# AnjieCheng/SpatialRGPT

Measured on AMD Instinct MI355X. Metric: region-grounded output tokens/sec @ VILA1.5-8B, 8 regions, greedy, higher is better.
Workload: dtype bf16; 1 GPU; BASELINE configs[1]: SpatialRGPT-VILA1.5-8B geometry (Llama-3-8B 32L/4096/GQA-8 + SigLIP-so400m 384px x2 passes + regiongpt extractor + mlp_downsample), 8 region masks, bs=1 per GPU, prompt 64 ids -> T=259, greedy 128 new tokens; parallelism=dp1, decode=hipGraph, llm_weights=bf16

## Files before the change

### include/srgpt.h

```cpp
#ifndef SRGPT_H_
#define SRGPT_H_

#include <stddef.h>
#include <stdint.h>

#ifdef __cplusplus
extern "C" {
#endif

typedef void* srgpt_stream_t;

enum { SRGPT_F32 = 0, SRGPT_BF16 = 1 };
enum { SRGPT_ACT_NONE = 0, SRGPT_ACT_GELU_ERF = 1, SRGPT_ACT_GELU_TANH = 2, SRGPT_ACT_SILU = 3, SRGPT_ACT_QUICK_GELU = 4 };
enum {
  SRGPT_OK = 0,
  SRGPT_ERR_ARG = -1,
  SRGPT_ERR_UNSUPPORTED = -2,
  SRGPT_ERR_LAUNCH = -3,
  SRGPT_ERR_STATE = -4
};
enum {
  SRGPT_OUT_PLAIN = 0,
  SRGPT_OUT_DECONV2X = 1
};
// ... 13 lines not shown
                    int64_t ws_bytes, int norm_kind, const void* norm_w, const void* norm_b, void* Y, float norm_eps, int dtype,
                    srgpt_stream_t stream);

int srgpt_gemm_swiglu(const void* A, const void* Wgu, void* out, int M, int I, int K, void* gu_scratch, void* ws,
                      int64_t ws_bytes, int dtype, srgpt_stream_t stream);

int srgpt_gemm_rope_kv_append(const void* A, const void* W, void* qkv, int K, void* ws, int64_t ws_bytes, void* kcache,
                              void* vcache, const int* pos0, const void* cos_tab, const void* sin_tab, int B, int T, int Hq,
                              int Hkv, int D, int max_pos, int dtype, srgpt_stream_t stream);

int srgpt_gemm_w8(const void* A, const void* W8, const float* wscale, const void* bias, const void* residual, void* C,
                  int M, int N, int K, int lda, int ldc, int act, int out_f32, void* ws, int64_t ws_bytes,
                  srgpt_stream_t stream);

int srgpt_quant_rows_e4m3(const void* x, void* q, float* scale, int M, int K, int ldx, srgpt_stream_t stream);
int srgpt_quant_rows_e4m3_rmsnorm(const void* x, const void* norm_w, float eps, void* q, float* scale, int M, int K, int ldx,
                                  srgpt_stream_t stream);
int srgpt_quant_rows_e4m3_swiglu(const void* gate_up, void* q, float* scale, int M, int inter, srgpt_stream_t stream);
int srgpt_gemm_w8a8(const void* A8, const float* ascale, const void* W8, const float* wscale, const void* bias,
                    const void* residual, void* C, int M, int N, int K, int lda, int ldc, int out_f32, void* ws,
                    int64_t ws_bytes, srgpt_stream_t stream);

int srgpt_gemv(const void* x, const void* W, const void* norm_w, float norm_eps, const void* residual,
               void* out, int batch, int N, int K, int swiglu, int out_f32, int dtype, srgpt_stream_t stream);
int srgpt_gemv_w8(const void* x, const void* W8, const float* wscale, const void* norm_w, float norm_eps,
                  const void* residual, void* out, int batch, int N, int K, int swiglu, int out_f32,
                  srgpt_stream_t stream);
#define SRGPT_ROWSS_STRIDE 512
int srgpt_gemv_rowss_supported(int batch, int dtype, int fp8);
int srgpt_gemv_rowss(const void* x, const void* W, const void* W8, const float* wscale, const void* norm_w, float norm_eps,
                     const void* residual, void* out, int batch, int N, int K, int swiglu, int out_f32, const float* rowss_in,
                     float* rowss_out, int packed_rows, srgpt_stream_t stream);
size_t srgpt_packed_bytes(int N, int K, int elem_bytes, int rows);
int srgpt_pack_decode_weights(const void* W, void* out, int N, int K, int elem_bytes, int rows, srgpt_stream_t stream);

int srgpt_layernorm(const void* x, const void* w, const void* b, void* y, int rows, int cols, float eps,
                    int act, int dtype, srgpt_stream_t stream);
int srgpt_rmsnorm(const void* x, const void* w, void* y, int rows, int cols, float eps, int dtype,
                  srgpt_stream_t stream);

int srgpt_attention(const void* q, const void* k, const void* v, void* o, int B, int Tq, int Tk, int Hq,
                    int Hkv, int D, int64_t q_bs, int64_t q_ts, int64_t q_hs, int64_t k_bs, int64_t k_ts,
                    int64_t k_hs, int64_t v_bs, int64_t v_ts, int64_t v_hs, float scale, int causal,
                    const int* kv_len, int dtype, srgpt_stream_t stream);

int srgpt_rope_kv_append(void* qkv, void* kcache, void* vcache, const int* pos0, const void* cos_tab,
                         const void* sin_tab, int B, int T, int Hq, int Hkv, int D, int max_pos, int dtype,
                         srgpt_stream_t stream);

int64_t srgpt_decode_attn_ws_floats(int B, int Hq, int D);
int srgpt_decode_attention(const void* qkv, void* kcache, void* vcache, const int* pos, const void* cos_tab,
                           const void* sin_tab, void* out, float* ws, int B, int Hq, int Hkv, int D,
                           int max_pos, int dtype, srgpt_stream_t stream);

int64_t srgpt_region_pool_ws_floats(int M, int fw, int C);
int srgpt_region_pool(const void* feat, const void* masks, void* out, float* ws, int M, int mh, int mw,
                      int fw, int C, float rscale_h, float rscale_w, int mask_dtype, int dtype,
                      srgpt_stream_t stream);
int srgpt_region_pool_u8(const void* feat, const void* masks_u8, const int* ys, const int* xs, void* out, float* ws, int M,
                         int rh, int rw, int mh, int mw, int fw, int C, float rscale_h, float rscale_w, int dtype,
                         srgpt_stream_t stream);
int srgpt_avgpool(const void* x, void* y, int n_img, int in_w, int out_w, int C, int dtype,
                  srgpt_stream_t stream);
int srgpt_s2d(const void* x, void* y, int n_img, int g, int C, int dtype, srgpt_stream_t stream);
int srgpt_im2col(const void* images, void* out, int n_img, int S, int patch, int kp, int dtype,
                 srgpt_stream_t stream);

int srgpt_embed_rows(const void* table, const int64_t* ids, void* out, int n, int cols, int dtype,
                     srgpt_stream_t stream);
#define SRGPT_SPLICE_STATS 8
int64_t srgpt_splice_scratch_ints(int B, int n_images_total);
int srgpt_splice_plan(const int64_t* ids, const unsigned char* attn_mask, int B, int P, int nimg_feat, int n_images_total,
                      const int* img_info, int use_masks, int use_depths, int64_t mask_id, int64_t depth_id, int max_len, int Tcap,
                      int* desc, int* stats, int* scratch, srgpt_stream_t stream);
int srgpt_splice_gather(const int* desc, const int* stats, int B, int Tcap, int T, int left_pad, int cols, int dtype,
                        const void* embed, const void* image_features, const void* mask_embeds, const void* depth_embeds,
                        const int64_t* labels, int P, int64_t ignore_index, void* out, int64_t* labels_out,
                        unsigned char* attn_mask_out, srgpt_stream_t stream);
int srgpt_kv_beam_reorder(void* kcache, void* vcache, const int64_t* beam_idx, int layers, int batch, int num_beams, int kv_heads,
                          int max_pos, int head_dim, int live, int dtype, srgpt_stream_t stream);
int srgpt_scatter_rows(const void* src, const int* src_idx, const int* idx, void* dst, int n, int cols,
                       int dtype, srgpt_stream_t stream);
int srgpt_silu_mul(const void* gu, void* out, int rows, int inter, int dtype, srgpt_stream_t stream);
int srgpt_argmax(const float* logits, int64_t* ids_out, int B, int V, srgpt_stream_t stream);
int srgpt_cross_entropy(const float* logits, const int64_t* labels, float* row_loss, float* out, int rows, int V,
                        int64_t ignore_index, srgpt_stream_t stream);


typedef struct {
  float temperature;
  int top_k;
  float top_p;
  float top_p_rm;
  uint64_t seed;
  uint64_t counter;
  int* kept_out;
} srgpt_sampling;

int64_t srgpt_sample_ws_bytes(int B);
int srgpt_sample(const float* logits, srgpt_sampling* sp, int64_t* tok_out, void* ws, int B, int V, srgpt_stream_t stream);
int srgpt_sample_status(const void* ws, int B, srgpt_stream_t stream);
int64_t srgpt_sample_full_ws_bytes(int B, int V);
int srgpt_sample_full(const float* logits, srgpt_sampling* sp, int64_t* tok_out, uint32_t* kept_mask, void* ws, int B, int V,
                      srgpt_stream_t stream);

typedef struct {
// ... 122 lines not shown
```

### spatialrgpt_amd/_lib.py

```python
from __future__ import annotations

import ctypes as C
import os
from typing import Optional

_HERE = os.path.dirname(os.path.abspath(__file__))
LIB_PATH = os.path.join(_HERE, "libsrgpt_hip.so")

F32, BF16 = 0, 1
ACT_NONE, ACT_GELU_ERF, ACT_GELU_TANH, ACT_SILU, ACT_QUICK_GELU = 0, 1, 2, 3, 4
OUT_PLAIN, OUT_DECONV2X = 0, 1
ERR_ARG, ERR_UNSUPPORTED, ERR_LAUNCH, ERR_STATE = -1, -2, -3, -4

vp, i32, i64, f32 = C.c_void_p, C.c_int, C.c_int64, C.c_float


class VitWeights(C.Structure):
    _fields_ = [
        ("dtype", i32), ("hidden", i32), ("inter", i32), ("heads", i32), ("n_layers_run", i32),
        ("image_size", i32), ("patch", i32), ("kp", i32), ("inter_pad", i32), ("act", i32), ("eps", f32),
        ("patch_w", vp), ("patch_b", vp), ("pos_emb", vp), ("cls_emb", vp), ("pre_ln_w", vp), ("pre_ln_b", vp),
        ("ln1_w", C.POINTER(vp)), ("ln1_b", C.POINTER(vp)),
        ("wqkv", C.POINTER(vp)), ("bqkv", C.POINTER(vp)),
        ("wo", C.POINTER(vp)), ("bo", C.POINTER(vp)),
# ... 28 lines not shown


class Sampling(C.Structure):
    _fields_ = [("temperature", f32), ("top_k", i32), ("top_p", f32), ("top_p_rm", f32), ("seed", C.c_uint64),
                ("counter", C.c_uint64), ("kept_out", vp)]


class LogitsProc(C.Structure):
    _fields_ = [("repetition_penalty", f32), ("no_repeat_ngram", i32), ("min_new_tokens", i32), ("n_eos", i32), ("eos", i64 * 8)]


LOGITS_PROC_EOS_MAX = 8
LOGITS_PROC_HISTORY_MAX = 12288
SAMPLING_TOP_K_MAX = 64
SAMPLING_KEPT_MAX = 256
SAMPLING_VOCAB_MAX = 128 * 2048
SAMPLER_TOPK64, SAMPLER_FULL = 0, 1

NORM_RMS, NORM_LAYER = 1, 2
SPLICE_STATS = 8
ROWSS_STRIDE = 512
ABI_VERSION = 9

_SIGNATURES = {
    "srgpt_last_error": (C.c_char_p, []),
    "srgpt_abi_version": (i32, []),
    "srgpt_device_cus": (i32, []),
    "srgpt_gemm_ws_bytes": (i64, [i32, i32]),
    "srgpt_gemm": (i32, [vp, vp, vp, vp, vp, i32, i32, i32, i32, i32, i32, i32, i32, i32, i32, i32, vp, i64, i32, vp]),
    "srgpt_gemm_norm": (i32, [vp, vp, vp, vp, vp, i32, i32, i32, vp, i64, i32, vp, vp, vp, f32, i32, vp]),
    "srgpt_gemm_rope_kv_append": (i32, [vp, vp, vp, i32, vp, i64, vp, vp, vp, vp, vp, i32, i32, i32, i32, i32, i32, i32, vp]),
    "srgpt_gemm_swiglu": (i32, [vp, vp, vp, i32, i32, i32, vp, vp, i64, i32, vp]),
    "srgpt_gemm_w8": (i32, [vp, vp, vp, vp, vp, vp, i32, i32, i32, i32, i32, i32, i32, vp, i64, vp]),
    "srgpt_quant_rows_e4m3": (i32, [vp, vp, vp, i32, i32, i32, vp]),
    "srgpt_quant_rows_e4m3_rmsnorm": (i32, [vp, vp, f32, vp, vp, i32, i32, i32, vp]),
    "srgpt_quant_rows_e4m3_swiglu": (i32, [vp, vp, vp, i32, i32, vp]),
    "srgpt_gemm_w8a8": (i32, [vp, vp, vp, vp, vp, vp, vp, i32, i32, i32, i32, i32, i32, vp, i64, vp]),
    "srgpt_gemv": (i32, [vp, vp, vp, f32, vp, vp, i32, i32, i32, i32, i32, i32, vp]),
    "srgpt_gemv_w8": (i32, [vp, vp, vp, vp, f32, vp, vp, i32, i32, i32, i32, i32, vp]),
    "srgpt_splice_scratch_ints": (i64, [i32, i32]),
    "srgpt_splice_plan": (i32, [vp, vp, i32, i32, i32, i32, vp, i32, i32, i64, i64, i32, i32, vp, vp, vp, vp]),
    "srgpt_splice_gather": (i32, [vp, vp, i32, i32, i32, i32, i32, i32, vp, vp, vp, vp, vp, i32, i64, vp, vp, vp, vp]),
    "srgpt_gemv_rowss_supported": (i32, [i32, i32, i32]),
    "srgpt_gemv_rowss": (i32, [vp, vp, vp, vp, vp, f32, vp, vp, i32, i32, i32, i32, i32, vp, vp, i32, vp]),
    "srgpt_packed_bytes": (C.c_size_t, [i32, i32, i32, i32]),
    "srgpt_pack_decode_weights": (i32, [vp, vp, i32, i32, i32, i32, vp]),
    "srgpt_layernorm": (i32, [vp, vp, vp, vp, i32, i32, f32, i32, i32, vp]),
    "srgpt_rmsnorm": (i32, [vp, vp, vp, i32, i32, f32, i32, vp]),
    "srgpt_attention": (i32, [vp, vp, vp, vp, i32, i32, i32, i32, i32, i32, i64, i64, i64, i64, i64, i64, i64, i64,
                              i64, f32, i32, vp, i32, vp]),
    "srgpt_rope_kv_append": (i32, [vp, vp, vp, vp, vp, vp, i32, i32, i32, i32, i32, i32, i32, vp]),
    "srgpt_decode_attn_ws_floats": (i64, [i32, i32, i32]),
    "srgpt_decode_attention": (i32, [vp, vp, vp, vp, vp, vp, vp, vp, i32, i32, i32, i32, i32, i32, vp]),
    "srgpt_region_pool_ws_floats": (i64, [i32, i32, i32]),
    "srgpt_region_pool": (i32, [vp, vp, vp, vp, i32, i32, i32, i32, i32, f32, f32, i32, i32, vp]),
    "srgpt_region_pool_u8": (i32, [vp, vp, vp, vp, vp, vp, i32, i32, i32, i32, i32, i32, i32, f32, f32, i32, vp]),
    "srgpt_avgpool": (i32, [vp, vp, i32, i32, i32, i32, i32, vp]),
    "srgpt_s2d": (i32, [vp, vp, i32, i32, i32, i32, vp]),
    "srgpt_im2col": (i32, [vp, vp, i32, i32, i32, i32, i32, vp]),
    "srgpt_embed_rows": (i32, [vp, vp, vp, i32, i32, i32, vp]),
    "srgpt_kv_beam_reorder": (i32, [vp, vp, vp, i32, i32, i32, i32, i32, i32, i32, i32, vp]),
    "srgpt_scatter_rows": (i32, [vp, vp, vp, vp, i32, i32, i32, vp]),
    "srgpt_silu_mul": (i32, [vp, vp, i32, i32, i32, vp]),
    "srgpt_argmax": (i32, [vp, vp, i32, i32, vp]),
    "srgpt_cross_entropy": (i32, [vp, vp, vp, vp, i32, i32, i64, vp]),
    "srgpt_sample_ws_bytes": (i64, [i32]),
    "srgpt_sample": (i32, [vp, vp, vp, vp, i32, i32, vp]),
    "srgpt_sample_status": (i32, [vp, i32, vp]),
    "srgpt_sample_full_ws_bytes": (i64, [i32, i32]),
    "srgpt_sample_full": (i32, [vp, vp, vp, vp, vp, i32, i32, vp]),
    "srgpt_logits_process": (i32, [vp, vp, vp, i32, i32, vp, i32, i32, vp]),
    "srgpt_image_resize_normalize": (i32, [vp, i32, i32, i32, vp, vp, i32, vp, vp, i32, i32, i32, vp, vp, vp, vp, f32, i32, i32, vp]),
    "srgpt_mask_resize_nearest": (i32, [vp, i32, i32, i32, vp, vp, i32, i32, vp, i32, vp]),
    "srgpt_mask_pad_resize": (i32, [vp, i32, i32, i32, vp, vp, i32, vp, vp, i32, i32, i32, vp, vp, i32, vp]),
    "srgpt_vit_assemble_cls": (i32, [vp, vp, vp, vp, i32, i32, i32, i32, vp]),
    "srgpt_vit_ws_bytes": (i64, [C.POINTER(VitWeights), i32]),
    "srgpt_vit_forward": (i32, [C.POINTER(VitWeights), vp, vp, vp, i32, vp]),
    "srgpt_llm_ws_bytes": (i64, [C.POINTER(LlmWeights), i32, i32]),
    "srgpt_llm_prefill": (i32, [C.POINTER(LlmWeights), C.POINTER(LlmState), vp, i32, vp, vp, vp]),
    "srgpt_llm_prefill_ragged": (i32, [C.POINTER(LlmWeights), C.POINTER(LlmState), vp, i32, vp, vp, vp, vp]),
    "srgpt_llm_decode_step": (i32, [C.POINTER(LlmWeights), C.POINTER(LlmState), vp]),
    "srgpt_llm_sample_first": (i32, [C.POINTER(LlmWeights), C.POINTER(LlmState), vp]),
    "srgpt_llm_decode_sync_state": (i32, [C.POINTER(LlmWeights), C.POINTER(LlmState), vp]),
    "srgpt_llm_decode_graph_create": (i32, [C.POINTER(LlmWeights), C.POINTER(LlmState), vp, C.POINTER(vp)]),
    "srgpt_llm_sample_first_ex": (i32, [C.POINTER(LlmWeights), C.POINTER(LlmState), i32, vp]),
    "srgpt_llm_decode_step_ex": (i32, [C.POINTER(LlmWeights), C.POINTER(LlmState), i32, vp]),
    "srgpt_llm_decode_graph_create_ex": (i32, [C.POINTER(LlmWeights), C.POINTER(LlmState), i32, vp, C.POINTER(vp)]),
    "srgpt_llm_sample_first_proc": (i32, [C.POINTER(LlmWeights), C.POINTER(LlmState), i32, vp, vp]),
    "srgpt_llm_decode_step_proc": (i32, [C.POINTER(LlmWeights), C.POINTER(LlmState), i32, vp, vp]),
    "srgpt_llm_decode_graph_create_proc": (i32, [C.POINTER(LlmWeights), C.POINTER(LlmState), i32, vp, vp, C.POINTER(vp)]),
    "srgpt_graph_launch": (i32, [vp, i32, vp]),
    "srgpt_graph_destroy": (i32, [vp]),
}

EXPORTED_SYMBOLS = tuple(_SIGNATURES)

_lib: Optional[C.CDLL] = None


class SrgptNativeError(RuntimeError):
    pass


def load() -> C.CDLL:
    global _lib
    if _lib is not None:
# ... 37 lines not shown
```

### spatialrgpt_amd/csrc/attn.hip

```cpp
#include <stdlib.h>

#include <type_traits>

#include "attn_route.h"
#include "common.h"
#include "internal.h"

namespace {

template <typename T>
__global__ __launch_bounds__(64) void simple_attn_kernel(const T* __restrict__ q, const T* __restrict__ k,
                                                         const T* __restrict__ v, T* __restrict__ o, int Tq, int Tk,
                                                         int Hq, int Hkv, int D, int64_t q_bs, int64_t q_ts,
                                                         int64_t q_hs, int64_t k_bs, int64_t k_ts, int64_t k_hs,
                                                         int64_t v_bs, int64_t v_ts, int64_t v_hs, float scale,
                                                         int causal, const int* __restrict__ kv_len) {
  __shared__ float qs[256];
  const int t = blockIdx.x, h = blockIdx.y, b = blockIdx.z, lane = threadIdx.x;
  const int hk = h / (Hq / Hkv);
  const int klen = kv_len ? min(kv_len[b], Tk) : Tk;
  const T* qp = q + b * q_bs + (int64_t)t * q_ts + h * q_hs;
  for (int d = lane; d < D; d += 64) qs[d] = to_f(qp[d]);
  __syncthreads();
  const T* kb = k + b * k_bs + hk * k_hs;
// ... 473 lines not shown
    if (lq < G && g4 == 0) wm[wave][lq] = alpha;
    asm volatile("s_waitcnt lgkmcnt(0)" ::: "memory");
    __builtin_amdgcn_wave_barrier();
#pragma unroll
    for (int h = 0; h < G; ++h) {
      const float a_h = wm[wave][h];
      acc[h][0] *= a_h;
      acc[h][1] *= a_h;
    }
#pragma unroll
    for (int i = 0; i < 16; ++i) {
      const int key = kb + i;
      unsigned int vv = vreg[i];
      if (key == P) vv = vnw;
      if (key >= kend) vv = 0u;
      const float v0 = bf16lo(vv), v1 = bf16hi(vv);
#pragma unroll
      for (int h = 0; h < G; ++h) {
        const float ph = pw[wave][i][h];
        acc[h][0] = fmaf(ph, v0, acc[h][0]);
        acc[h][1] = fmaf(ph, v1, acc[h][1]);
      }
    }
    asm volatile("s_waitcnt lgkmcnt(0)" ::: "memory");
    __builtin_amdgcn_wave_barrier();
    if (kb + 64 < kend) fetch(kb + 64);
  }
  if (lq < G && g4 == 0) {
    wm[wave][lq] = m_run;
    wl[wave][lq] = l_run;
  }
#pragma unroll
  for (int h = 0; h < G; ++h) *reinterpret_cast<f32x2*>(&accs[wave][h][2 * lane]) = f32x2{acc[h][0], acc[h][1]};
  __syncthreads();
  float* wbase = ws + attn_ws_group(b, hk, Hkv, G, D);
  const PublishPartial publish;
  for (int w = tid; w < G * (D / 2); w += 256) {
    const int gq = w / (D / 2), d = 2 * (w - gq * (D / 2));
    const float M = fmaxf(fmaxf(wm[0][gq], wm[1][gq]), fmaxf(wm[2][gq], wm[3][gq]));
    float n0 = 0.f, n1 = 0.f, L = 0.f;
#pragma unroll
    for (int wv = 0; wv < 4; ++wv) {
      const float e = (wm[wv][gq] > -INFINITY) ? __expf(wm[wv][gq] - M) : 0.f;
      n0 = fmaf(e, accs[wv][gq][d], n0);
      n1 = fmaf(e, accs[wv][gq][d + 1], n1);
      L = fmaf(e, wl[wv][gq], L);
    }
    float* wp = wbase + attn_ws_row(gq, split, D);
    publish(wp + d, n0, n1);
    if (d == 0) publish(wp + D, M, L);
  }
  decode_ticket_merge<T, D, G, 64>(wbase, attn_ws_ticket(tickets, b, hk, Hkv), nlive, out + ((size_t)b * Hq + (size_t)hk * G) * D,
                                   &sc[0][0], stat_m, stat_l, tid, lane, wave);
}

template <typename T>
int launch_decode(const void* qkv, void* kc, void* vc, const int* pos, const void* ct, const void* st, void* out,
                  float* ws, int B, int Hq, int Hkv, int D, int max_pos, const DecodePrefetch& pf, hipStream_t s) {
  const AttnDecodeRoute r = attn_decode_route(std::is_same<T, bf16_t>::value, B, Hq, Hkv, D, max_pos, srgpt_device_cus());
  SRGPT_CHECK(r.status != ATTN_MAX_POS_TOO_LONG, SRGPT_ERR_UNSUPPORTED, "srgpt_decode_attention: max_pos %d exceeds %d cached positions",
              max_pos, ATTN_DEC_SPLIT_MAX * ATTN_DEC_CHUNK_MAX);
  SRGPT_CHECK(r.status != ATTN_BAD_HEAD_DIM, SRGPT_ERR_UNSUPPORTED, "srgpt_decode_attention: head_dim %d not supported (16,32,64,128)", D);
  SRGPT_CHECK(r.status != ATTN_BAD_GROUP, SRGPT_ERR_UNSUPPORTED, "srgpt_decode_attention: heads/kv_heads = %d not supported (1,2,4,8)",
              r.G);
  const float scale = 1.0f / sqrtf((float)D);
  int* tickets = reinterpret_cast<int*>(ws + attn_ws_partial_floats(B, Hq, D));
  const dim3 grid(r.n_attn + (pf.base ? pf.nblocks : 0)), block(256);
  int rc = SRGPT_OK;
  if constexpr (std::is_same<T, bf16_t>::value) {
    if (r.family == ATTN_DECODE_MFMA)
      rc = srgpt_switch<1, 2, 4, 8>(r.G, "heads/kv_heads", [&](auto g_c) {
        hipLaunchKernelGGL((decode_mfma_kernel<decltype(g_c)::value>), grid, block, 0, s, (const T*)qkv, (T*)kc, (T*)vc, pos,
                           (const T*)ct, (const T*)st, ws, tickets, (T*)out, Hq, Hkv, max_pos, r.nsplit, r.kpb, scale, r.n_attn, pf);
        return (int)SRGPT_OK;
      });
  }
  if (r.family == ATTN_DECODE_VALU)
    rc = srgpt_switch<16, 32, 64, 128>(D, "head_dim", [&](auto d_c) {
      return srgpt_switch<1, 2, 4, 8>(r.G, "heads/kv_heads", [&](auto g_c) {
        hipLaunchKernelGGL((decode_split_kernel<T, decltype(d_c)::value, decltype(g_c)::value>), grid, block, 0, s, (const T*)qkv,
                           (T*)kc, (T*)vc, pos, (const T*)ct, (const T*)st, ws, tickets, (T*)out, Hq, Hkv, max_pos, r.nsplit, scale,
                           r.n_attn, pf);
        return (int)SRGPT_OK;
      });
    });
  SRGPT_TRY(rc);
  SRGPT_LAUNCH_CHECK();
  return SRGPT_OK;
}

}

extern "C" int64_t srgpt_decode_attn_ws_floats(int B, int Hq, int D) {
  return (int64_t)attn_ws_floats(B, Hq, D);
}

int srgpt_decode_attention_pf(const void* qkv, void* kcache, void* vcache, const int* pos, const void* cos_tab,
                              const void* sin_tab, void* out, float* ws, int B, int Hq, int Hkv, int D, int max_pos, int dtype,
                              const void* next_w, int next_n, int next_k, int next_fp8, srgpt_stream_t stream) {
  SRGPT_CHECK(qkv && kcache && vcache && pos && cos_tab && sin_tab && out && ws, SRGPT_ERR_ARG,
              "srgpt_decode_attention: null pointer");
  SRGPT_CHECK(B > 0 && Hq > 0 && Hkv > 0 && Hq % Hkv == 0, SRGPT_ERR_ARG, "srgpt_decode_attention: bad heads");
  const DecodePrefetch pf = srgpt_prefetch_for_gemv(dtype == SRGPT_BF16 ? next_w : nullptr, next_n, next_k, next_fp8, B);
  if (dtype == SRGPT_BF16)
    return launch_decode<bf16_t>(qkv, kcache, vcache, pos, cos_tab, sin_tab, out, ws, B, Hq, Hkv, D, max_pos, pf,
                                 as_stream(stream));
  if (dtype == SRGPT_F32)
    return launch_decode<float>(qkv, kcache, vcache, pos, cos_tab, sin_tab, out, ws, B, Hq, Hkv, D, max_pos, pf,
                                as_stream(stream));
  srgpt_set_error("srgpt_decode_attention: bad dtype %d", dtype);
  return SRGPT_ERR_ARG;
}

void* srgpt_decode_attn_sync_words(float* ws, int B, int Hq, int D, size_t* bytes) {
  if (bytes) *bytes = attn_ws_tickets_reserved(B, Hq) * sizeof(int);
  return ws + attn_ws_partial_floats(B, Hq, D);
}

extern "C" int srgpt_decode_attention(const void* qkv, void* kcache, void* vcache, const int* pos, const void* cos_tab,
                                      const void* sin_tab, void* out, float* ws, int B, int Hq, int Hkv, int D,
                                      int max_pos, int dtype, srgpt_stream_t stream) {
  return srgpt_decode_attention_pf(qkv, kcache, vcache, pos, cos_tab, sin_tab, out, ws, B, Hq, Hkv, D, max_pos, dtype, nullptr, 0,
                                   0, 0, stream);
}

extern "C" int srgpt_attention(const void* q, const void* k, const void* v, void* o, int B, int Tq, int Tk, int Hq,
                               int Hkv, int D, int64_t q_bs, int64_t q_ts, int64_t q_hs, int64_t k_bs, int64_t k_ts,
                               int64_t k_hs, int64_t v_bs, int64_t v_ts, int64_t v_hs, float scale, int causal,
                               const int* kv_len, int dtype, srgpt_stream_t stream) {
  SRGPT_CHECK(q && k && v && o, SRGPT_ERR_ARG, "srgpt_attention: null pointer");
  SRGPT_CHECK(B > 0 && Tq > 0 && Tk > 0 && Hq > 0 && Hkv > 0 && Hq % Hkv == 0 && D > 0 && D <= 256, SRGPT_ERR_ARG,
              "srgpt_attention: bad shape B=%d Tq=%d Tk=%d Hq=%d Hkv=%d D=%d", B, Tq, Tk, Hq, Hkv, D);
  SRGPT_CHECK(dtype == SRGPT_BF16 || dtype == SRGPT_F32, SRGPT_ERR_ARG, "srgpt_attention: bad dtype %d", dtype);
  hipStream_t s = as_stream(stream);
  const bool qkv16 = (uintptr_t)q % 16 == 0 && (uintptr_t)k % 16 == 0 && (uintptr_t)v % 16 == 0;
  const AttnPrefillRoute r = attn_prefill_route(dtype == SRGPT_BF16, D, Tq, Tk, Hq, B, q_bs, q_ts, q_hs, k_bs, k_ts, k_hs, v_bs, v_ts, v_hs,
                                                qkv16, (uintptr_t)o % 8 == 0, scale > 0.f);
  const dim3 grid(r.grid_x, r.grid_y, r.grid_z), block(r.block);
  if (r.family == ATTN_FLASH) {
    AttnArgs a{(const bf16_t*)q, (const bf16_t*)k, (const bf16_t*)v, (bf16_t*)o, Tq, Tk, Hq, Hkv, D,
               q_bs, q_ts, q_hs, k_bs, k_ts, k_hs, v_bs, v_ts, v_hs, scale, kv_len};
    SRGPT_TRY(srgpt_flash_bf16_launch(a, r, causal != 0, s));
  } else if (dtype == SRGPT_BF16) {
    hipLaunchKernelGGL(simple_attn_kernel<bf16_t>, grid, block, 0, s, (const bf16_t*)q, (const bf16_t*)k, (const bf16_t*)v, (bf16_t*)o,
                       Tq, Tk, Hq, Hkv, D, q_bs, q_ts, q_hs, k_bs, k_ts, k_hs, v_bs, v_ts, v_hs, scale, causal, kv_len);
  } else {
    hipLaunchKernelGGL(simple_attn_kernel<float>, grid, block, 0, s, (const float*)q, (const float*)k, (const float*)v, (float*)o, Tq,
                       Tk, Hq, Hkv, D, q_bs, q_ts, q_hs, k_bs, k_ts, k_hs, v_bs, v_ts, v_hs, scale, causal, kv_len);
  }
  SRGPT_LAUNCH_CHECK();
  return SRGPT_OK;
}
```

### spatialrgpt_amd/csrc/attn_route.h

```cpp
#pragma once
#include <stddef.h>
#include <stdint.h>

enum AttnFamily {
  ATTN_FLASH,
  ATTN_ONE_WAVE,
  ATTN_DECODE_MFMA,
  ATTN_DECODE_VALU,
};

enum AttnStatus {
  ATTN_OK,
  ATTN_MAX_POS_TOO_LONG,
  ATTN_BAD_HEAD_DIM,
  ATTN_BAD_GROUP,
};

struct AttnPrefillRoute {
  AttnFamily family;
  int hdp;
  int grid_x, grid_y, grid_z, block;
};

struct AttnDecodeRoute {
// ... 25 lines not shown
namespace attn_route_detail {

constexpr int ceil_div(int a, int b) { return (a + b - 1) / b; }

constexpr bool decode_use_mfma(bool bf16, int D, int G) { return bf16 && D == 128 && (G == 1 || G == 2 || G == 4 || G == 8); }

constexpr int decode_nsplit_mfma(int max_pos) {
  int n = ceil_div(max_pos, ATTN_DEC_MFMA_KEYS);
  if (n < 1) n = 1;
  if (n > ATTN_DEC_SPLIT_MAX) n = ATTN_DEC_SPLIT_MAX;
  return n;
}

constexpr int decode_nsplit_valu(int max_pos, int B, int Hkv, int cus) {
  int want = ceil_div(2 * cus, Hkv * B);
  const int cap = B == 1 ? 16 : 8;
  if (want > cap) want = cap;
  if (want < 1) want = 1;
  int n = ceil_div(max_pos, ATTN_DEC_CHUNK_MAX);
  if (n < want) n = want;
  if (n > ATTN_DEC_SPLIT_MAX) n = ATTN_DEC_SPLIT_MAX;
  return n;
}

}

inline AttnPrefillRoute attn_prefill_route(bool bf16, int D, int Tq, int Tk, int Hq, int B, int64_t q_bs, int64_t q_ts, int64_t q_hs,
                                           int64_t k_bs, int64_t k_ts, int64_t k_hs, int64_t v_bs, int64_t v_ts, int64_t v_hs,
                                           bool qkv_aligned16, bool o_aligned8, bool scale_positive) {
  const bool vec_ok = D % 8 == 0 && D <= 128 && q_ts % 8 == 0 && q_hs % 8 == 0 && q_bs % 8 == 0 && k_ts % 8 == 0 && k_hs % 8 == 0 &&
                      k_bs % 8 == 0 && v_ts % 8 == 0 && v_hs % 8 == 0 && v_bs % 8 == 0 && qkv_aligned16 && o_aligned8;
  const int64_t span = ((int64_t)Tk + 4 * 64) * (k_ts > v_ts ? k_ts : v_ts) * 2;
  if (bf16 && vec_ok && scale_positive && span < ATTN_FLASH_SLICE_SPAN_LIMIT)
    return AttnPrefillRoute{ATTN_FLASH, (D + 31) / 32 * 32, attn_route_detail::ceil_div(Tq, ATTN_FLASH_QBLK), Hq, B, 256};
  return AttnPrefillRoute{ATTN_ONE_WAVE, 0, Tq, Hq, B, 64};
}

inline AttnDecodeRoute attn_decode_route(bool bf16, int B, int Hq, int Hkv, int D, int max_pos, int cus) {
  using namespace attn_route_detail;
  AttnDecodeRoute r{ATTN_OK, ATTN_DECODE_VALU, Hq / Hkv, 0, 0, 0};
  if (decode_use_mfma(bf16, D, r.G)) {
    r.family = ATTN_DECODE_MFMA;
    r.nsplit = decode_nsplit_mfma(max_pos);
    r.kpb = ceil_div(ceil_div(max_pos, r.nsplit), ATTN_DEC_MFMA_KEYS) * ATTN_DEC_MFMA_KEYS;
  } else {
    r.nsplit = decode_nsplit_valu(max_pos, B, Hkv, cus);
  }
  r.n_attn = Hkv * r.nsplit * B;
  if (r.family == ATTN_DECODE_VALU && ceil_div(max_pos, r.nsplit) > ATTN_DEC_CHUNK_MAX) r.status = ATTN_MAX_POS_TOO_LONG;
  else if (D != 16 && D != 32 && D != 64 && D != 128) r.status = ATTN_BAD_HEAD_DIM;
  else if (r.G != 1 && r.G != 2 && r.G != 4 && r.G != 8) r.status = ATTN_BAD_GROUP;
  return r;
}
```

### spatialrgpt_amd/csrc/common.h

```cpp
#pragma once
#include <hip/hip_runtime.h>
#include <stdint.h>
#include <stdio.h>
#include <string.h>

#include <type_traits>

#include "../../include/srgpt.h"
#include "gemv_route.h"

typedef __bf16 bf16_t;
typedef __attribute__((ext_vector_type(8))) __bf16 bf16x8;
typedef __attribute__((ext_vector_type(4))) __bf16 bf16x4;
typedef __attribute__((ext_vector_type(2))) __bf16 bf16x2;
typedef __attribute__((ext_vector_type(4))) float f32x4;
typedef __attribute__((ext_vector_type(2))) float f32x2;
typedef __attribute__((ext_vector_type(16))) float f32x16;
typedef __attribute__((ext_vector_type(4))) unsigned int u32x4;
typedef __attribute__((ext_vector_type(2))) unsigned int u32x2;

#define WAVE 64

void srgpt_set_error(const char* fmt, ...);

// ... 149 lines not shown
  static constexpr int N = 8;
  bf16x8 v;
  __device__ __forceinline__ float get(int i) const { return (float)v[i]; }
  __device__ __forceinline__ void set(int i, float x) { v[i] = (bf16_t)x; }
};

__device__ __forceinline__ float gelu_erf(float x) { return 0.5f * x * (1.f + erff(x * 0.70710678118654752440f)); }
__device__ __forceinline__ float gelu_tanh(float x) {
  const float k0 = 0.7978845608028654f, k1 = 0.044715f;
  return 0.5f * x * (1.f + tanhf(k0 * (x + k1 * x * x * x)));
}
__device__ __forceinline__ float silu(float x) { return x / (1.f + __expf(-x)); }

template <typename T>
__device__ __forceinline__ float apply_act(float x, int act) {
  switch (act) {
    case SRGPT_ACT_GELU_ERF: return gelu_erf(x);
    case SRGPT_ACT_GELU_TANH: return gelu_tanh(x);
    case SRGPT_ACT_SILU: return silu(x);
    case SRGPT_ACT_QUICK_GELU: return x / (1.f + __expf(-1.702f * x));
    default: return x;
  }
}

struct SrgptPrefetch {
  const char* base;
  long long row_bytes;
  int n_units;
  int unit_rows;
  int umul, rstride;
  int gemv_grid;
  int nblocks;
  int n_rows;
};
constexpr int SRGPT_PREFETCH_ROUNDS = 2;

template <int NB>
__device__ __forceinline__ void srgpt_prefetch_rows(const SrgptPrefetch& pf, int p, int wave, int lane) {
  const int per_row = (int)(pf.row_bytes >> 10);
  int done = 0;
  for (int u = p * 4 + wave; u < pf.n_units && done < SRGPT_PREFETCH_ROUNDS; u += pf.gemv_grid * 4, ++done)
    for (int r = 0; r < pf.unit_rows; ++r) {
      const long long ri = min((long long)u * pf.umul + (long long)r * pf.rstride, (long long)pf.n_rows - 1);
      const char* row = pf.base + (size_t)ri * pf.row_bytes + lane * 16;
      for (int c0 = 0; c0 < per_row; c0 += NB) {
        u32x4 v[NB];
#pragma unroll
        for (int c = 0; c < NB; ++c) v[c] = *reinterpret_cast<const u32x4*>(row + ((size_t)min(c0 + c, per_row - 1) << 10));
#pragma unroll
        for (int c = 0; c < NB; ++c) asm volatile("" ::"v"(v[c]));
      }
    }
}
__device__ __forceinline__ void srgpt_prefetch_block(const SrgptPrefetch& pf, int p, int wave, int lane) {
  srgpt_prefetch_rows<2>(pf, p, wave, lane);
}

extern "C" int srgpt_device_cus(void);
static inline SrgptPrefetch srgpt_prefetch_for_gemv(const void* W, int N, int K, int fp8, int batch) {
  SrgptPrefetch pf{nullptr, 0, 0, 1, 1, 0, 1, 0, 0};
  const long long row_bytes = fp8 ? (long long)K : 2LL * K;
  if (!W || batch > 1 || row_bytes % 1024 != 0) return pf;
  const GemvFamily family = gemv_route(1, K, true, fp8 != 0, false).family;
  if (family == GEMV_SKINNY) return pf;
  const int grid = gemv_valu_launch(family, 1, N, K, true, false, srgpt_device_cus()).grid;
  pf.base = reinterpret_cast<const char*>(W);
  pf.row_bytes = row_bytes;
  pf.n_units = fp8 ? (N + 1) / 2 : N;
  pf.unit_rows = fp8 ? 2 : 1;
  pf.umul = fp8 ? 2 : 1;
  pf.rstride = fp8 ? 1 : N;
  pf.gemv_grid = grid;
  pf.nblocks = grid;
  pf.n_rows = N;
  return pf;
}
```

### spatialrgpt_amd/ops.py

```python
from __future__ import annotations

import ctypes as C
import math
from typing import Optional

import torch

from . import _lib as L

_DT = {torch.float32: L.F32, torch.bfloat16: L.BF16}


def dt_code(t: torch.Tensor) -> int:
    try:
        return _DT[t.dtype]
    except KeyError:
        raise ValueError(f"srgpt kernels support float32 and bfloat16 tensors, got {t.dtype}") from None


def _p(t: Optional[torch.Tensor]):
    return None if t is None else t.data_ptr()


def _stream():
# ... 268 lines not shown
    assert q.stride(3) == 1 and k.stride(3) == 1 and v.stride(3) == 1
    if scale is None:
        scale = 1.0 / math.sqrt(D)
    o = torch.empty((B, Tq, Hq, D), device=q.device, dtype=q.dtype)
    L.check(L.load().srgpt_attention(_p(q), _p(k), _p(v), _p(o), B, Tq, Tk, Hq, Hkv, D, q.stride(0), q.stride(1),
                                     q.stride(2), k.stride(0), k.stride(1), k.stride(2), v.stride(0), v.stride(1),
                                     v.stride(2), float(scale), int(causal), _p(kv_len), dt_code(q), _stream()))
    return o


def gemm_swiglu(a, wgu, out=None):
    _dev(a, wgu)
    _same_dtype("gemm_swiglu", a, weight=wgu)
    M, K = a.shape
    I = wgu.shape[0] // 2
    assert wgu.shape == (2 * I, K) and a.is_contiguous() and wgu.is_contiguous()
    if out is None:
        out = torch.empty((M, I), device=a.device, dtype=a.dtype)
    scratch = torch.empty((M, 2 * I), device=a.device, dtype=a.dtype)
    ws, ws_bytes = _ws_arg(a.device, M, 2 * I, a.dtype == torch.bfloat16)
    L.check(L.load().srgpt_gemm_swiglu(_p(a), _p(wgu), _p(out), M, I, K, _p(scratch), ws, ws_bytes,
                                       dt_code(a), _stream()))
    return out


def gemm_rope_kv_append(a, w, kcache, vcache, cos_tab, sin_tab, B, T, Hq, Hkv, D, pos0=None, qkv=None):
    _dev(a, w, kcache, vcache, cos_tab, sin_tab)
    M, K = a.shape
    N = (Hq + 2 * Hkv) * D
    assert M == B * T and w.shape == (N, K) and a.is_contiguous() and w.is_contiguous()
    if qkv is None:
        qkv = torch.empty((M, N), device=a.device, dtype=a.dtype)
    ws, ws_bytes = _ws_arg(a.device, M, N, a.dtype == torch.bfloat16)
    max_pos = kcache.shape[-2]
    L.check(L.load().srgpt_gemm_rope_kv_append(_p(a), _p(w), _p(qkv), K, ws, ws_bytes, _p(kcache),
                                               _p(vcache), _p(pos0), _p(cos_tab), _p(sin_tab), B, T, Hq, Hkv, D, max_pos,
                                               dt_code(a), _stream()))
    return qkv


def rope_kv_append(qkv, kcache, vcache, cos_tab, sin_tab, B, T, Hq, Hkv, D, pos0=None):
    _dev(qkv, kcache, vcache, cos_tab, sin_tab)
    max_pos = kcache.shape[-2]
    L.check(L.load().srgpt_rope_kv_append(_p(qkv), _p(kcache), _p(vcache), _p(pos0), _p(cos_tab), _p(sin_tab), B, T, Hq,
                                          Hkv, D, max_pos, dt_code(qkv), _stream()))


def decode_attention_ws(B, Hq, D, device):
    n = int(L.load().srgpt_decode_attn_ws_floats(B, Hq, D))
    ws = torch.zeros((n,), device=device, dtype=torch.float32)
    return ws, ws[B * Hq * 64 * (D + 2):].view(torch.int32)


def decode_attention(qkv, kcache, vcache, pos, cos_tab, sin_tab, Hq, Hkv, D, ws=None):
    _dev(qkv, kcache, vcache, pos)
    B = qkv.shape[0]
    max_pos = kcache.shape[-2]
    out = torch.empty((B, Hq * D), device=qkv.device, dtype=qkv.dtype)
    if ws is None:
        ws = decode_attention_ws(B, Hq, D, qkv.device)[0]
    else:
        _dev(ws)
        assert ws.dtype == torch.float32 and ws.is_contiguous() and ws.numel() >= L.load().srgpt_decode_attn_ws_floats(B, Hq, D)
    L.check(L.load().srgpt_decode_attention(_p(qkv), _p(kcache), _p(vcache), _p(pos), _p(cos_tab), _p(sin_tab), _p(out),
                                            _p(ws), B, Hq, Hkv, D, max_pos, dt_code(qkv), _stream()))
    return out


def region_pool(feat, masks, fw: Optional[int] = None):
    _dev(feat, masks)
    Lf, Cc = feat.shape
    M, mh, mw = masks.shape
    sf = (Lf / (mh * mw)) ** 0.5
    oh, ow = int(math.floor(mh * sf)), int(math.floor(mw * sf))
    if oh * ow != Lf or oh != ow:
        raise RuntimeError(f"mask of size {mh}x{mw} resamples to {oh}x{ow}, which does not match {Lf} feature tokens")
    if masks.dtype not in (torch.float32, torch.bfloat16):
        masks = masks.float()
    masks = _c(masks)
    rs = 1.0 / sf
    outs = []
    lib = L.load()
    for m0 in range(0, M, 16):
        mm = min(16, M - m0)
        out = torch.empty((mm, Cc), device=feat.device, dtype=feat.dtype)
        ws = torch.empty((lib.srgpt_region_pool_ws_floats(mm, oh, Cc),), device=feat.device, dtype=torch.float32)
        L.check(lib.srgpt_region_pool(_p(_c(feat)), _p(masks[m0:m0 + mm]), _p(out), _p(ws), mm, mh, mw, oh, Cc, rs, rs,
                                      _DT[masks.dtype], dt_code(feat), _stream()))
        outs.append(out)
    return outs[0] if len(outs) == 1 else torch.cat(outs, dim=0)


def region_pool_u8(feat, masks_u8, size: int):
    from .mm_utils import cv2_nearest_index

    _dev(feat, masks_u8)
    if masks_u8.dtype != torch.uint8 or masks_u8.dim() != 3:
        raise ValueError("region_pool_u8: masks must be a uint8 tensor [M, H, W]")
    Lf, Cc = feat.shape
    M, rh, rw = masks_u8.shape
    mh = mw = int(size)
    sf = (Lf / (mh * mw)) ** 0.5
    oh, ow = int(math.floor(mh * sf)), int(math.floor(mw * sf))
    if oh * ow != Lf or oh != ow:
        raise RuntimeError(f"mask of size {mh}x{mw} resamples to {oh}x{ow}, which does not match {Lf} feature tokens")
    ys = torch.from_numpy(cv2_nearest_index(rh, mh)).to(feat.device)
    xs = torch.from_numpy(cv2_nearest_index(rw, mw)).to(feat.device)
    masks_u8 = _c(masks_u8)
    rs = 1.0 / sf
    lib = L.load()
    outs = []
    for m0 in range(0, M, 16):
        mm = min(16, M - m0)
        out = torch.empty((mm, Cc), device=feat.device, dtype=feat.dtype)
        ws = torch.empty((lib.srgpt_region_pool_ws_floats(mm, oh, Cc),), device=feat.device, dtype=torch.float32)
        L.check(lib.srgpt_region_pool_u8(_p(_c(feat)), _p(masks_u8[m0:m0 + mm]), _p(ys), _p(xs), _p(out), _p(ws), mm, rh, rw, mh, mw,
                                         oh, Cc, rs, rs, dt_code(feat), _stream()))
        outs.append(out)
    return outs[0] if len(outs) == 1 else torch.cat(outs, dim=0)
# ... 204 lines not shown
```

Before: 336.4 tokens/s.

## Add single-block-per-head fused decode attention kernel for short KV caches

New measurement: 334.2 tokens/s. No clear change (-0.6%).

```diff
diff --git a/include/srgpt.h b/include/srgpt.h
--- a/include/srgpt.h
+++ b/include/srgpt.h
@@ -89,6 +89,9 @@
 int srgpt_decode_attention(const void* qkv, void* kcache, void* vcache, const int* pos, const void* cos_tab,
                            const void* sin_tab, void* out, float* ws, int B, int Hq, int Hkv, int D,
                            int max_pos, int dtype, srgpt_stream_t stream);
+int srgpt_decode_attention_block(const void* qkv, void* kcache, void* vcache, const int* pos, const void* cos_tab,
+                                 const void* sin_tab, void* out, float* ws, int B, int Hq, int Hkv, int D,
+                                 int max_pos, int dtype, srgpt_stream_t stream);
 
 int64_t srgpt_region_pool_ws_floats(int M, int fw, int C);
 int srgpt_region_pool(const void* feat, const void* masks, void* out, float* ws, int M, int mh, int mw,
diff --git a/spatialrgpt_amd/_lib.py b/spatialrgpt_amd/_lib.py
--- a/spatialrgpt_amd/_lib.py
+++ b/spatialrgpt_amd/_lib.py
@@ -104,6 +104,7 @@
     "srgpt_rope_kv_append": (i32, [vp, vp, vp, vp, vp, vp, i32, i32, i32, i32, i32, i32, i32, vp]),
     "srgpt_decode_attn_ws_floats": (i64, [i32, i32, i32]),
     "srgpt_decode_attention": (i32, [vp, vp, vp, vp, vp, vp, vp, vp, i32, i32, i32, i32, i32, i32, vp]),
+    "srgpt_decode_attention_block": (i32, [vp, vp, vp, vp, vp, vp, vp, vp, i32, i32, i32, i32, i32, i32, vp]),
     "srgpt_region_pool_ws_floats": (i64, [i32, i32, i32]),
     "srgpt_region_pool": (i32, [vp, vp, vp, vp, i32, i32, i32, i32, i32, f32, f32, i32, i32, vp]),
     "srgpt_region_pool_u8": (i32, [vp, vp, vp, vp, vp, vp, i32, i32, i32, i32, i32, i32, i32, f32, f32, i32, vp]),
diff --git a/spatialrgpt_amd/csrc/attn.hip b/spatialrgpt_amd/csrc/attn.hip
--- a/spatialrgpt_amd/csrc/attn.hip
+++ b/spatialrgpt_amd/csrc/attn.hip
@@ -549,6 +549,212 @@
   }
   decode_ticket_merge<T, D, G, 64>(wbase, attn_ws_ticket(tickets, b, hk, Hkv), nlive, out + ((size_t)b * Hq + (size_t)hk * G) * D,
                                    &sc[0][0], stat_m, stat_l, tid, lane, wave);
+}
+
+constexpr int DB_WAVES = ATTN_DEC_BLOCK_THREADS / 64;
+constexpr int DB_PASS_MAX = ATTN_DEC_BLOCK_MAX_POS / ATTN_DEC_BLOCK_KEYS;
+constexpr int DB_SPLIT_MAX = ATTN_DEC_BLOCK_MAX_POS / ATTN_DEC_MFMA_KEYS;
+static_assert(ATTN_DEC_BLOCK_KEYS == 16 * DB_WAVES && DB_SPLIT_MAX <= 64, "a wave owns 16 keys of a pass; one lane per split in the merge");
+
+struct DecodeBlockRows {
+  u32x4 k[4];
+  unsigned int v[16];
+};
+
+__device__ __forceinline__ float lane_value(float x, int src_lane) {
+  return __builtin_bit_cast(float, __builtin_amdgcn_readlane(__builtin_bit_cast(int, x), src_lane));
+}
+
+__global__ __launch_bounds__(ATTN_DEC_BLOCK_THREADS) void decode_block_kernel(
+    const bf16_t* __restrict__ qkv, bf16_t* __restrict__ kcache, bf16_t* __restrict__ vcache, const int* __restrict__ pos,
+    const bf16_t* __restrict__ cos_tab, const bf16_t* __restrict__ sin_tab, bf16_t* __restrict__ out, int Hq, int Hkv, int max_pos,
+    float scale, int n_attn, DecodePrefetch pf) {
+  typedef bf16_t T;
+  constexpr int D = 128, HALF = 64;
+  __shared__ __attribute__((aligned(16))) bf16_t qs[16 * DM_QLD];
+  __shared__ __attribute__((aligned(16))) bf16_t knew[D], vnew[D];
+  __shared__ __attribute__((aligned(16))) float accs[DB_PASS_MAX * DB_WAVES][D];
+  __shared__ float wm[DB_PASS_MAX * DB_WAVES], wl[DB_PASS_MAX * DB_WAVES];
+  __shared__ __attribute__((aligned(16))) float part[DB_SPLIT_MAX][D];
+  __shared__ float pm[DB_SPLIT_MAX], pl[DB_SPLIT_MAX];
+
+  const int tid = threadIdx.x, lane = tid & 63, wave = __builtin_amdgcn_readfirstlane(tid >> 6);
+  if ((int)blockIdx.x >= n_attn) {
+    const int q = (int)blockIdx.x - n_attn;
+    const int p = ((q >> 3) * 4 + (wave >> 2)) * 8 + ((int)blockIdx.x & 7);
+    if (p < pf.nblocks) srgpt_prefetch_block(pf, p, wave & 3, lane);
+    return;
+  }
+  const int G = Hq / Hkv;
+  const int b = (int)blockIdx.x / Hq, j_blk = (int)blockIdx.x % Hq;
+  const int hk = j_blk % Hkv, gq = j_blk / Hkv, h = hk * G + gq;
+  const int P = pos[b];
+  const int total = P + 1;
+  const int npass = min((total + ATTN_DEC_BLOCK_KEYS - 1) / ATTN_DEC_BLOCK_KEYS, DB_PASS_MAX);
+  const int nlive = min((total + ATTN_DEC_MFMA_KEYS - 1) / ATTN_DEC_MFMA_KEYS, DB_SPLIT_MAX);
+  const T* row = qkv + (size_t)b * (Hq + 2 * Hkv) * D;
+  T* kc = kcache + ((size_t)b * Hkv + hk) * (size_t)max_pos * D;
+  T* vc = vcache + ((size_t)b * Hkv + hk) * (size_t)max_pos * D;
+  const int lq = lane & 15, g4 = lane >> 4;
+
+  auto fetch = [&](DecodeBlockRows& r, int kb) {
+    if (kb < P) {
+      const T* kr = kc + (size_t)min(kb + lq, P - 1) * D + g4 * 8;
+#pragma unroll
+      for (int j = 0; j < 4; ++j) r.k[j] = *reinterpret_cast<const u32x4*>(kr + 32 * j);
+#pragma unroll
+      for (int i = 0; i < 16; ++i) r.v[i] = *reinterpret_cast<const unsigned int*>(vc + (size_t)min(kb + i, P - 1) * D + 2 * lane);
+    } else {
+#pragma unroll
+      for (int j = 0; j < 4; ++j) r.k[j] = u32x4{0u, 0u, 0u, 0u};
+#pragma unroll
+      for (int i = 0; i < 16; ++i) r.v[i] = 0u;
+    }
+  };
+  DecodeBlockRows ra, rb;
+  const int kb0 = 16 * wave;
+  fetch(ra, kb0);
+  if (npass > 1) fetch(rb, kb0 + ATTN_DEC_BLOCK_KEYS);
+
+  if (wave <= G) {
+    const int i = lane;
+    const T* p = wave < G ? row + (size_t)(hk * G + wave) * D : row + (size_t)(Hq + hk) * D;
+    const float x1 = to_f(p[i]), x2 = to_f(p[i + HALF]);
+    const float c = to_f(cos_tab[(size_t)P * HALF + i]), s = to_f(sin_tab[(size_t)P * HALF + i]);
+    const T o1 = from_f<T>(rnd<T>(x1 * c) + rnd<T>(-x2 * s));
+    const T o2 = from_f<T>(rnd<T>(x2 * c) + rnd<T>(x1 * s));
+    T* dst = wave < G ? qs + wave * DM_QLD : knew;
+    dst[i] = o1;
+    dst[i + HALF] = o2;
+  } else if (wave == G + 1) {
+    *reinterpret_cast<unsigned int*>(vnew + 2 * lane) = *reinterpret_cast<const unsigned int*>(row + (size_t)(Hq + Hkv + hk) * D + 2 * lane);
+  }
+  for (int i = tid; i < (16 - G) * (D / 2); i += ATTN_DEC_BLOCK_THREADS) {
+    const int r = G + i / (D / 2), c = 2 * (i % (D / 2));
+    *reinterpret_cast<unsigned int*>(qs + r * DM_QLD + c) = 0u;
+  }
+  __syncthreads();
+  if (gq == 0 && tid < D / 2) {
+    *reinterpret_cast<unsigned int*>(kc + (size_t)P * D + 2 * tid) = *reinterpret_cast<const unsigned int*>(knew + 2 * tid);
+    *reinterpret_cast<unsigned int*>(vc + (size_t)P * D + 2 * tid) = *reinterpret_cast<const unsigned int*>(vnew + 2 * tid);
+  }
+  bf16x8 qf[4];
+#pragma unroll
+  for (int j = 0; j < 4; ++j) qf[j] = *reinterpret_cast<const bf16x8*>(qs + lq * DM_QLD + 32 * j + g4 * 8);
+  const unsigned int vnw = *reinterpret_cast<const unsigned int*>(vnew + 2 * lane);
+
+  auto compute = [&](DecodeBlockRows& r, int kb, int slot) {
+    float m_run = -INFINITY, l_run = 0.f, a0 = 0.f, a1 = 0.f;
+    if (kb < total) {
+      const int kend = total;
+      if ((unsigned)(P - kb) < 16u) {
+#pragma unroll
+        for (int j = 0; j < 4; ++j) {
+          const u32x4 kn = *reinterpret_cast<const u32x4*>(knew + 32 * j + g4 * 8);
+          if (kb + lq == P) r.k[j] = kn;
+        }
+      }
+      f32x4 sacc = {0.f, 0.f, 0.f, 0.f};
+#pragma unroll
+      for (int j = 0; j < 4; ++j) sacc = __builtin_amdgcn_mfma_f32_16x16x32_bf16(__builtin_bit_cast(bf16x8, r.k[j]), qf[j], sacc, 0, 0, 0);
+      float sv4[4], mx = -INFINITY;
+#pragma unroll
+      for (int rr = 0; rr < 4; ++rr) {
+        const int key = kb + 4 * g4 + rr;
+        sv4[rr] = key < kend ? sacc[rr] * scale : -INFINITY;
+        mx = fmaxf(mx, sv4[rr]);
+      }
+      mx = rows_pair(mx, [](float a, float b2) { return fmaxf(a, b2); });
+      mx = halves_pair(mx, [](float a, float b2) { return fmaxf(a, b2); });
+      m_run = mx;
+      float rs = 0.f;
+      f32x4 pv;
+#pragma unroll
+      for (int rr = 0; rr < 4; ++rr) {
+        pv[rr] = __expf(sv4[rr] - m_run);
+        rs += pv[rr];
+      }
+      rs = rows_pair(rs, [](float a, float b2) { return a + b2; });
+      rs = halves_pair(rs, [](float a, float b2) { return a + b2; });
+      l_run = rs;
+#pragma unroll
+      for (int i = 0; i < 16; ++i) {
+        const int key = kb + i;
+        unsigned int vv = r.v[i];
+        if (key == P) vv = vnw;
+        if (key >= kend) vv = 0u;
+        const float ph = lane_value(pv[i & 3], 16 * (i >> 2) + gq);
+        a0 = fmaf(ph, bf16lo(vv), a0);
+        a1 = fmaf(ph, bf16hi(vv), a1);
+      }
+    }
+    if (lane == gq) {
+      wm[slot] = m_run;
+      wl[slot] = l_run;
+    }
+    *reinterpret_cast<f32x2*>(&accs[slot][2 * lane]) = f32x2{a0, a1};
+  };
+  static_assert(DB_PASS_MAX == 4, "the four passes are written out");
+  compute(ra, kb0, wave);
+  if (npass > 2) fetch(ra, kb0 + 2 * ATTN_DEC_BLOCK_KEYS);
+  if (npass > 1) {
+    compute(rb, kb0 + ATTN_DEC_BLOCK_KEYS, DB_WAVES + wave);
+    if (npass > 3) fetch(rb, kb0 + 3 * ATTN_DEC_BLOCK_KEYS);
+    if (npass > 2) compute(ra, kb0 + 2 * ATTN_DEC_BLOCK_KEYS, 2 * DB_WAVES + wave);
+    if (npass > 3) compute(rb, kb0 + 3 * ATTN_DEC_BLOCK_KEYS, 3 * DB_WAVES + wave);
+  }
+  __syncthreads();
+  if (wave < nlive) {
+    const float* m4 = wm + 4 * wave;
+    const float M = fmaxf(fmaxf(m4[0], m4[1]), fmaxf(m4[2], m4[3]));
+    float n0 = 0.f, n1 = 0.f, L = 0.f;
+#pragma unroll
+    for (int wv = 0; wv < 4; ++wv) {
+      const float e = (m4[wv] > -INFINITY) ? __expf(m4[wv] - M) : 0.f;
+      const f32x2 x = *reinterpret_cast<const f32x2*>(&accs[4 * wave + wv][2 * lane]);
+      n0 = fmaf(e, x[0], n0);
+      n1 = fmaf(e, x[1], n1);
+      L = fmaf(e, wl[4 * wave + wv], L);
+    }
+    *reinterpret_cast<f32x2*>(&part[wave][2 * lane]) = f32x2{n0, n1};
+    if (lane == 0) {
+      pm[wave] = M;
+      pl[wave] = L;
+    }
+  }
+  __syncthreads();
+  if (wave != 0) return;
+  const bool ok = lane < nlive;
+  const int sidx = ok ? lane : nlive - 1;
+  const float ms = ok ? pm[sidx] : -INFINITY;
+  const float ls = ok ? pl[sidx] : 0.f;
+  const float Mx = lanes_max<64>(ms);
+  const float wv = (ms > -INFINITY) ? __expf(ms - Mx) : 0.f;
+  const float den = lanes_sum<64>(wv * ls);
+  const float inv = den > 0.f ? 1.f / den : 0.f;
+  float n0 = 0.f, n1 = 0.f;
+#pragma unroll
+  for (int j = 0; j < DB_SPLIT_MAX; ++j)
+    if (j < nlive) {
+      const float wj = lane_value(wv, j);
+      const f32x2 x = *reinterpret_cast<const f32x2*>(&part[j][2 * lane]);
+      n0 = fmaf(wj, x[0], n0);
+      n1 = fmaf(wj, x[1], n1);
+    }
+  T* op = out + ((size_t)b * Hq + h) * D + 2 * lane;
+  op[0] = from_f<T>(n0 * inv);
+  op[1] = from_f<T>(n1 * inv);
+}
+
+int launch_decode_block(const AttnDecodeBlockRoute& r, const void* qkv, void* kc, void* vc, const int* pos, const void* ct,
+                        const void* st, void* out, int Hq, int Hkv, int D, int max_pos, const DecodePrefetch& pf, hipStream_t s) {
+  typedef bf16_t T;
+  const float scale = 1.0f / sqrtf((float)D);
+  const int n_pf = pf.base ? (pf.nblocks + 31) / 32 * 8 : 0;
+  hipLaunchKernelGGL(decode_block_kernel, dim3(r.n_attn + n_pf), dim3(ATTN_DEC_BLOCK_THREADS), 0, s, (const T*)qkv, (T*)kc, (T*)vc, pos,
+                     (const T*)ct, (const T*)st, (T*)out, Hq, Hkv, max_pos, scale, r.n_attn, pf);
+  SRGPT_LAUNCH_CHECK();
+  return SRGPT_OK;
 }
 
 template <typename T>
@@ -592,21 +798,38 @@
   return (int64_t)attn_ws_floats(B, Hq, D);
 }
 
+namespace {
+
+enum DecodeWhich { DECODE_PINNED, DECODE_BLOCK_FIRST, DECODE_BLOCK_ONLY };
+
+int decode_attention_impl(DecodeWhich which, const void* qkv, void* kcache, void* vcache, const int* pos, const void* cos_tab,
+                          const void* sin_tab, void* out, float* ws, int B, int Hq, int Hkv, int D, int max_pos, int dtype,
+                          const void* next_w, int next_n, int next_k, int next_fp8, srgpt_stream_t stream) {
+  SRGPT_CHECK(qkv && kcache && vcache && pos && cos_tab && sin_tab && out && ws, SRGPT_ERR_ARG,
+              "srgpt_decode_attention: null pointer");
+  SRGPT_CHECK(B > 0 && Hq > 0 && Hkv > 0 && Hq % Hkv == 0, SRGPT_ERR_ARG, "srgpt_decode_attention: bad heads");
+  SRGPT_CHECK(dtype == SRGPT_BF16 || dtype == SRGPT_F32, SRGPT_ERR_ARG, "srgpt_decode_attention: bad dtype %d", dtype);
+  const DecodePrefetch pf = srgpt_prefetch_for_gemv(dtype == SRGPT_BF16 ? next_w : nullptr, next_n, next_k, next_fp8, B);
+  if (which != DECODE_PINNED) {
+    const AttnDecodeBlockRoute r = attn_decode_block_route(dtype == SRGPT_BF16, B, Hq, Hkv, D, max_pos);
+    if (r.serves)
+      return launch_decode_block(r, qkv, kcache, vcache, pos, cos_tab, sin_tab, out, Hq, Hkv, D, max_pos, pf, as_stream(stream));
+    SRGPT_CHECK(which != DECODE_BLOCK_ONLY, SRGPT_ERR_UNSUPPORTED,
+                "srgpt_decode_attention_block: serves bf16, head_dim 128, heads/kv_heads 1,2,4,8 and max_pos <= %d", ATTN_DEC_BLOCK_MAX_POS);
+  }
+  if (dtype == SRGPT_BF16)
+    return launch_decode<bf16_t>(qkv, kcache, vcache, pos, cos_tab, sin_tab, out, ws, B, Hq, Hkv, D, max_pos, pf,
+                                 as_stream(stream));
+  return launch_decode<float>(qkv, kcache, vcache, pos, cos_tab, sin_tab, out, ws, B, Hq, Hkv, D, max_pos, pf, as_stream(stream));
+}
+
+}
+
 int srgpt_decode_attention_pf(const void* qkv, void* kcache, void* vcache, const int* pos, const void* cos_tab,
                               const void* sin_tab, void* out, float* ws, int B, int Hq, int Hkv, int D, int max_pos, int dtype,
                               const void* next_w, int next_n, int next_k, int next_fp8, srgpt_stream_t stream) {
-  SRGPT_CHECK(qkv && kcache && vcache && pos && cos_tab && sin_tab && out && ws, SRGPT_ERR_ARG,
-              "srgpt_decode_attention: null pointer");
-  SRGPT_CHECK(B > 0 && Hq > 0 && Hkv > 0 && Hq % Hkv == 0, SRGPT_ERR_ARG, "srgpt_decode_attention: bad heads");
-  const DecodePrefetch pf = srgpt_prefetch_for_gemv(dtype == SRGPT_BF16 ? next_w : nullptr, next_n, next_k, next_fp8, B);
-  if (dtype == SRGPT_BF16)
-    return launch_decode<bf16_t>(qkv, kcache, vcache, pos, cos_tab, sin_tab, out, ws, B, Hq, Hkv, D, max_pos, pf,
-                                 as_stream(stream));
-  if (dtype == SRGPT_F32)
-    return launch_decode<float>(qkv, kcache, vcache, pos, cos_tab, sin_tab, out, ws, B, Hq, Hkv, D, max_pos, pf,
-                                as_stream(stream));
-  srgpt_set_error("srgpt_decode_attention: bad dtype %d", dtype);
-  return SRGPT_ERR_ARG;
+  return decode_attention_impl(DECODE_BLOCK_FIRST, qkv, kcache, vcache, pos, cos_tab, sin_tab, out, ws, B, Hq, Hkv, D, max_pos, dtype,
+                               next_w, next_n, next_k, next_fp8, stream);
 }
 
 void* srgpt_decode_attn_sync_words(float* ws, int B, int Hq, int D, size_t* bytes) {
@@ -617,8 +840,15 @@
 extern "C" int srgpt_decode_attention(const void* qkv, void* kcache, void* vcache, const int* pos, const void* cos_tab,
                                       const void* sin_tab, void* out, float* ws, int B, int Hq, int Hkv, int D,
                                       int max_pos, int dtype, srgpt_stream_t stream) {
-  return srgpt_decode_attention_pf(qkv, kcache, vcache, pos, cos_tab, sin_tab, out, ws, B, Hq, Hkv, D, max_pos, dtype, nullptr, 0,
-                                   0, 0, stream);
+  return decode_attention_impl(DECODE_PINNED, qkv, kcache, vcache, pos, cos_tab, sin_tab, out, ws, B, Hq, Hkv, D, max_pos, dtype,
+                               nullptr, 0, 0, 0, stream);
+}
+
+extern "C" int srgpt_decode_attention_block(const void* qkv, void* kcache, void* vcache, const int* pos, const void* cos_tab,
+                                            const void* sin_tab, void* out, float* ws, int B, int Hq, int Hkv, int D,
+                                            int max_pos, int dtype, srgpt_stream_t stream) {
+  return decode_attention_impl(DECODE_BLOCK_ONLY, qkv, kcache, vcache, pos, cos_tab, sin_tab, out, ws, B, Hq, Hkv, D, max_pos, dtype,
+                               nullptr, 0, 0, 0, stream);
 }
 
 extern "C" int srgpt_attention(const void* q, const void* k, const void* v, void* o, int B, int Tq, int Tk, int Hq,
diff --git a/spatialrgpt_amd/csrc/attn_route.h b/spatialrgpt_amd/csrc/attn_route.h
--- a/spatialrgpt_amd/csrc/attn_route.h
+++ b/spatialrgpt_amd/csrc/attn_route.h
@@ -101,3 +101,24 @@
   else if (r.G != 1 && r.G != 2 && r.G != 4 && r.G != 8) r.status = ATTN_BAD_GROUP;
   return r;
 }
+
+constexpr int ATTN_DEC_BLOCK_THREADS = 1024;
+constexpr int ATTN_DEC_BLOCK_KEYS = 256;
+constexpr int ATTN_DEC_BLOCK_MAX_POS = 1024;
+
+struct AttnDecodeBlockRoute {
+  bool serves;
+  int G;
+  int n_attn;
+  int max_passes;
+};
+
+inline AttnDecodeBlockRoute attn_decode_block_route(bool bf16, int B, int Hq, int Hkv, int D, int max_pos) {
+  using namespace attn_route_detail;
+  AttnDecodeBlockRoute r{false, Hq / Hkv, 0, 0};
+  if (!decode_use_mfma(bf16, D, r.G) || max_pos < 1 || max_pos > ATTN_DEC_BLOCK_MAX_POS) return r;
+  r.serves = true;
+  r.n_attn = B * Hq;
+  r.max_passes = ceil_div(max_pos, ATTN_DEC_BLOCK_KEYS);
+  return r;
+}
diff --git a/spatialrgpt_amd/csrc/common.h b/spatialrgpt_amd/csrc/common.h
--- a/spatialrgpt_amd/csrc/common.h
+++ b/spatialrgpt_amd/csrc/common.h
@@ -225,8 +225,9 @@
       }
     }
 }
+constexpr int SRGPT_PREFETCH_INFLIGHT = 2;
 __device__ __forceinline__ void srgpt_prefetch_block(const SrgptPrefetch& pf, int p, int wave, int lane) {
-  srgpt_prefetch_rows<2>(pf, p, wave, lane);
+  srgpt_prefetch_rows<SRGPT_PREFETCH_INFLIGHT>(pf, p, wave, lane);
 }
 
 extern "C" int srgpt_device_cus(void);
diff --git a/spatialrgpt_amd/ops.py b/spatialrgpt_amd/ops.py
--- a/spatialrgpt_amd/ops.py
+++ b/spatialrgpt_amd/ops.py
@@ -344,7 +344,7 @@
     return ws, ws[B * Hq * 64 * (D + 2):].view(torch.int32)
 
 
-def decode_attention(qkv, kcache, vcache, pos, cos_tab, sin_tab, Hq, Hkv, D, ws=None):
+def decode_attention(qkv, kcache, vcache, pos, cos_tab, sin_tab, Hq, Hkv, D, ws=None, entry="srgpt_decode_attention"):
     _dev(qkv, kcache, vcache, pos)
     B = qkv.shape[0]
     max_pos = kcache.shape[-2]
@@ -354,9 +354,13 @@
     else:
         _dev(ws)
         assert ws.dtype == torch.float32 and ws.is_contiguous() and ws.numel() >= L.load().srgpt_decode_attn_ws_floats(B, Hq, D)
-    L.check(L.load().srgpt_decode_attention(_p(qkv), _p(kcache), _p(vcache), _p(pos), _p(cos_tab), _p(sin_tab), _p(out),
-                                            _p(ws), B, Hq, Hkv, D, max_pos, dt_code(qkv), _stream()))
-    return out
+    L.check(getattr(L.load(), entry)(_p(qkv), _p(kcache), _p(vcache), _p(pos), _p(cos_tab), _p(sin_tab), _p(out), _p(ws), B, Hq, Hkv,
+                                     D, max_pos, dt_code(qkv), _stream()))
+    return out
+
+
+def decode_attention_block(qkv, kcache, vcache, pos, cos_tab, sin_tab, Hq, Hkv, D, ws=None):
+    return decode_attention(qkv, kcache, vcache, pos, cos_tab, sin_tab, Hq, Hkv, D, ws, entry="srgpt_decode_attention_block")
 
 
 def region_pool(feat, masks, fw: Optional[int] = None):
```
